# andimarafioti/faster-qwen3-tts

Measured on AMD Instinct MI355X. Metric: real-time factor (audio s / wall s), Qwen3-TTS-12Hz-0.6B voice-clone streaming chunk_size=8; p50 TTFA in ttfa_ms_p50, higher is better.
Workload: dtype bf16

## Files before the change

faster-qwen3-tts_amd/csrc/decode_kernels.cuh:

```cuda
#pragma once
#include "fq3_common.cuh"
#include <initializer_list>

namespace fq3 {

enum { PRO_PLAIN = 0, PRO_NORM = 1, PRO_COMBINE = 2 };
enum { EPI_STORE = 0, EPI_RESIDUAL = 1, EPI_SWIGLU = 2 };

constexpr int kHeadDim = 128;
constexpr int kKeysPerTile = 64;
constexpr int kMaxWorkers = 8;
constexpr int kPartStride = kHeadDim + 4;


struct GemvArgs {
    const void* W; int N; int K;
    const void* x;
    const void* norm_w; float eps;
    const void* bias;
    void* y;
    const void* res;
    void* xn_out;
    int up_off;
    const float* part; int n_part; int rep;
// ... 680 lines not shown
                       a.n_kv, a.rep, a.max_seq, a.pos_imm, attn_tail(a));
}

template <typename T>
__global__ __launch_bounds__(256) void rmsnorm_kernel(const T* x, const T* w, T* y, int K, float eps) {
    __shared__ float red[8];
    float ss = 0.f;
    for (int e = threadIdx.x; e < K; e += 256) { const float v = DT<T>::ld(x + e); ss = fmaf(v, v, ss); }
    ss = block_sum<4>(ss, red);
    const float rs = 1.0f / sqrtf(ss / (float)K + eps);
    for (int e = threadIdx.x; e < K; e += 256)
        DT<T>::st(y + e, DT<T>::ld(w + e) * DT<T>::rnd(DT<T>::ld(x + e) * rs));
}

template <typename T>
__global__ void copy_kernel(T* dst, const T* src, int n) {
    const int i = blockIdx.x * blockDim.x + threadIdx.x;
    if (i < n) dst[i] = src[i];
}

struct DecodeState {
    int token, frame, pos, gen_step, done;
    int text_open;
    int min_new, max_new, trailing_len, noise_frames, eos_id, max_seq, sup_lo, sup_hi;
    float t_temperature; int t_top_k; float t_top_p; int t_do_sample; float t_rep_penalty;
    float p_temperature; int p_top_k; float p_top_p; int p_do_sample;
    const void* trailing_text; const void* tts_pad; const void* talker_noise; const void* pred_noise;
    const void* past_hidden_init;
    int n_pad, rope_delta;
};

struct TeacherForcing { const int* forced; int* decisions; };

__device__ __forceinline__ int forced_or(const TeacherForcing* tf, int slot, int tok) {
    if (!tf) return tok;
    const int* forced = gptr(tf->forced); int* dec = gptr(tf->decisions);
    if (dec && threadIdx.x == 0) dec[slot] = tok;
    return forced ? forced[slot] : tok;
}

template <typename T>
__device__ __forceinline__ void frame_begin_body(DecodeState* st, const T* codec_emb, const T* past_hidden, T* ph_hold,
                                                 T* pred_in, int* codes, unsigned char* seen, int H, int G) {
    const int done = st->done;
    if (done == 1) return;
    const int tok = st->token;
    if (tok == st->eos_id || st->frame >= st->max_new) {
        __syncthreads();
        if (threadIdx.x == 0) st->done = 1;
        return;
    }
    if (st->text_open && st->gen_step >= st->trailing_len) {
        if (done == 0) {
            for (int e = threadIdx.x; e < H; e += 256) ph_hold[e] = past_hidden[e];
            __syncthreads();
            if (threadIdx.x == 0) st->done = 2;
        }
        return;
    }
    if (done == 2) {
        past_hidden = ph_hold;
        __syncthreads();
        if (threadIdx.x == 0) st->done = 0;
    }
    if (threadIdx.x == 0) { codes[(size_t)st->frame * G] = tok; seen[tok] = 1; }
    for (int e = threadIdx.x; e < H; e += 256) {
        pred_in[e] = past_hidden[e];
        pred_in[H + e] = codec_emb[(size_t)tok * H + e];
    }
}
// ... 72 lines not shown
```

faster-qwen3-tts_amd/csrc/fq3_api.hip:

```cpp
#define FQ3_SKINNY_EXTERN
#include "fq3_ctx.h"
#include "sampler.cuh"
#include "sampler_wave.cuh"
#include "skinny_gemm.cuh"
#include "state_kernels.cuh"

#include <cstdio>
#include <cstdlib>
#include <cstring>
#include <map>
#include <string>
#include <type_traits>
#include <vector>

using namespace fq3;

static thread_local std::string g_err;
static int fail(int code, const std::string& m) { g_err = m; return code; }
int fq3_fail_(int code, const std::string& m) { return fail(code, m); }
#define HIPCHK(x) do { hipError_t e_ = (x); if (e_ != hipSuccess) return fail(FQ3_EHIP, std::string(#x) + ": " + hipGetErrorString(e_)); } while (0)

extern "C" const char* fq3_last_error(void) { return g_err.c_str(); }
extern "C" void fq3_set_error_(const char* msg) { g_err = msg ? msg : ""; }
extern "C" int fq3_abi_version(void) { return FQ3_ABI_VERSION; }
// ... 190 lines not shown
    if ((r = dmalloc(c, &c->pred_x2, (size_t)p.hidden * c->esz))) return r;
    if ((r = dmalloc(c, &c->xin, (size_t)Hm * c->esz))) return r;
    if ((r = dmalloc(c, &c->tmp_hidden, (size_t)Hm * c->esz))) return r;
    if ((r = dmalloc(c, &c->qkv, (size_t)qkvm * c->esz))) return r;
    if ((r = dmalloc(c, &c->act, (size_t)Im * c->esz))) return r;
    if ((r = dmalloc(c, &c->logits, (size_t)Vm * c->esz))) return r;
    if ((r = dmalloc(c, &c->past_hidden, (size_t)t.hidden * c->esz))) return r;
    if ((r = dmalloc(c, &c->ph_hold, (size_t)t.hidden * c->esz))) return r;
    if ((r = dmalloc(c, &c->pred_in, (size_t)2 * t.hidden * c->esz))) return r;
    if ((r = dmalloc(c, &c->pred_next, (size_t)t.hidden * c->esz))) return r;
    if ((r = dmalloc(c, &c->pred_x, (size_t)p.hidden * c->esz))) return r;
    if ((r = dmalloc(c, &c->plogits, (size_t)(G - 1) * p.vocab * c->esz))) return r;
    const int maxkv = std::max(t.n_kv_heads, p.n_kv_heads);
    c->part_stride = (size_t)maxkv * kMaxWorkers * 4 * kPartStride;
    if ((r = dmalloc(c, (void**)&c->part, 2 * c->part_stride * sizeof(float)))) return r;
    if ((r = dmalloc(c, (void**)&c->rope_now, 2 * 64 * sizeof(float)))) return r;
    if ((r = dmalloc(c, (void**)&c->seen_api, kMaxVocab))) return r;
    if ((r = dmalloc(c, (void**)&c->st, sizeof(DecodeState)))) return r;
    if ((r = dmalloc(c, (void**)&c->seen, kMaxVocab))) return r;
    if ((r = dmalloc(c, (void**)&c->codes, (size_t)(frames + 1) * G * sizeof(int)))) return r;
    if ((r = dmalloc(c, (void**)&c->ids64, (size_t)64 * sizeof(int64_t)))) return r;
    if ((r = dmalloc(c, (void**)&c->d_pemb, (size_t)64 * sizeof(void*)))) return r;
    HIPCHK(hipStreamCreateWithFlags(&c->cap_stream, hipStreamNonBlocking));
    return FQ3_OK;
}

extern "C" int fq3_set_option(fq3_ctx* c, const char* key, int value) {
    if (!c || !key) return fail(FQ3_EINVAL, "null argument");
    const std::string k(key);
    if (k == "weight_nt") c->opt_nt = value;
    else if (k == "pred_m2") c->opt_m2 = value;
    else if (k == "pred_attn") c->opt_pred_attn = value;
    else if (k == "rows_per_wave_max") c->opt_rmax = value;
    else if (k == "prefill_mode") c->prefill_mode = value;
    else if (k == "flash_prefill") c->opt_flash_prefill = value;
    else if (k == "flash_small") c->opt_flash_small = value;
    else if (k == "cont_pack") c->opt_cont_pack = value;
    else if (k == "swiglu_tile") c->opt_swiglu_tile = value;
    else if (k == "packed_weights") c->opt_packed = value;
    else if (k == "skinny_gemm") c->opt_no_skinny = !value;
    else return fail(FQ3_EINVAL, "unknown option: " + k);
    fq3_graph_reset(c);
    return FQ3_OK;
}

extern "C" int fq3_graph_reset(fq3_ctx* c) {
    if (!c) return fail(FQ3_EINVAL, "null ctx");
    if (c->exec) { (void)hipGraphExecDestroy(c->exec); c->exec = nullptr; }
    if (c->graph) { (void)hipGraphDestroy(c->graph); c->graph = nullptr; }
    return FQ3_OK;
}

namespace {
struct PackedEntry { void* p; int refs; int N, K; };
std::mutex g_packed_mu;
std::map<std::pair<const void*, int>, PackedEntry> g_packed;
}
const void* fq3_packed_find_(const void* W, int kind) {
    std::lock_guard<std::mutex> lk(g_packed_mu);
    auto it = g_packed.find({W, kind});
    return it == g_packed.end() ? nullptr : it->second.p;
}
int fq3_packed_acquire_(const void* W, int N, int K, int kind) {
    if (!W || !skinny_pack_ok(N, K) || (kind == 1 && (N / 2) % 8) || (kind == 2 && N % 512)) return FQ3_EUNSUPPORTED;
    std::lock_guard<std::mutex> lk(g_packed_mu);
    auto it = g_packed.find({W, kind});
// ... 15 lines not shown
    if (it == g_packed.end()) return;
    if (--it->second.refs <= 0) { (void)hipFree(it->second.p); g_packed.erase(it); }
}
static void packed_release_all(fq3_ctx* c) {
    for (auto& r : c->packed_refs) fq3_packed_release_(r.first, r.second);
    c->packed_refs.clear();
}
static int packed_acquire_all(fq3_ctx* c) {
    if (c->cfg.dtype != FQ3_BF16) return FQ3_OK;
    auto take = [&](const void* W, int N, int K, int kind) -> int {
        const int r = fq3_packed_acquire_(W, N, K, kind);
        if (r == FQ3_OK) c->packed_refs.emplace_back(W, kind);
        return r == FQ3_EUNSUPPORTED ? FQ3_OK : r;
    };
    auto stack = [&](const std::vector<fq3_layer_weights>& L, const fq3_stack_dims& d) -> int {
        const int qd = d.n_heads * kHeadDim, kvd = d.n_kv_heads * kHeadDim;
        for (const fq3_layer_weights& l : L) {
            if (int r = take(l.qkv, qd + 2 * kvd, d.hidden, 0)) return r;
            if (int r = take(l.o, d.hidden, qd, 0)) return r;
            if (int r = take(l.gate_up, 2 * d.inter, d.hidden, 1)) return r;
            if (int r = take(l.gate_up, 2 * d.inter, d.hidden, 0)) return r;
            if (int r = take(l.down, d.hidden, d.inter, 0)) return r;
        }
        return FQ3_OK;
    };
    if (int r = stack(c->tl, c->cfg.talker)) return r;
    if (int r = stack(c->pl, c->cfg.predictor)) return r;
    for (const fq3_layer_weights& l : c->tl) if (int r = take(l.gate_up, 2 * c->cfg.talker.inter, c->cfg.talker.hidden, 2)) return r;
    if (int r = take(c->wt.codec_head, c->cfg.talker.vocab, c->cfg.talker.hidden, 0)) return r;
    for (const void* h : c->lmh) if (int r = take(h, c->cfg.predictor.vocab, c->cfg.predictor.hidden, 0)) return r;
    return FQ3_OK;
}

extern "C" int fq3_ctx_destroy(fq3_ctx* c) {
    if (!c) return FQ3_OK;
    (void)hipDeviceSynchronize();
    fq3_graph_reset(c);
    packed_release_all(c);
    if (c->cap_stream) (void)hipStreamDestroy(c->cap_stream);
    if (fq3_kv_pool* p = c->tk.pool) {
        (void)fq3_kv_release(c, 0);
        bool last;
        { std::lock_guard<std::mutex> lk(p->mu); last = --p->users == 0; }
        if (p->is_private && last) pool_free_(p);
    }
    for (void* p : c->allocs) (void)hipFree(p);
    delete c;
    return FQ3_OK;
}

extern "C" int fq3_bind_weights(fq3_ctx* c, const fq3_weight_table* w) {
    if (!c || !w) return fail(FQ3_EINVAL, "null argument");
    const int G = c->cfg.num_code_groups;
    if (!w->talker_layers || !w->predictor_layers || !w->codec_embedding || !w->codec_head || !w->talker_final_norm ||
        !w->predictor_final_norm || !w->predictor_embeddings || !w->lm_heads || !w->talker_cos || !w->talker_sin ||
        !w->pred_cos || !w->pred_sin)
        return fail(FQ3_EINVAL, "weight table has null entries");
    if (c->cfg.has_projection && !w->proj_w) return fail(FQ3_EINVAL, "has_projection set but proj_w is null");
    if (w->talker_rope_len < c->cfg.max_seq_len || w->pred_rope_len < G + 1)
        return fail(FQ3_EINVAL, "rope tables shorter than the caches");
    c->wt = *w;
    c->tl.assign(w->talker_layers, w->talker_layers + c->cfg.talker.n_layers);
    c->pl.assign(w->predictor_layers, w->predictor_layers + c->cfg.predictor.n_layers);
    c->pemb.assign(w->predictor_embeddings, w->predictor_embeddings + (G - 1));
    c->lmh.assign(w->lm_heads, w->lm_heads + (G - 1));
    for (auto& l : c->tl) if (!l.qkv || !l.o || !l.gate_up || !l.down || !l.input_norm || !l.post_norm || !l.q_norm || !l.k_norm)
        return fail(FQ3_EINVAL, "talker layer has null weights");
    for (auto& l : c->pl) if (!l.qkv || !l.o || !l.gate_up || !l.down || !l.input_norm || !l.post_norm || !l.q_norm || !l.k_norm)
        return fail(FQ3_EINVAL, "predictor layer has null weights");
    HIPCHK(hipMemcpy(c->d_pemb, c->pemb.data(), (G - 1) * sizeof(void*), hipMemcpyHostToDevice));
    (void)hipDeviceSynchronize();
    packed_release_all(c);
    if (int r = packed_acquire_all(c)) { packed_release_all(c); return r; }
    c->bound = true;
    fq3_graph_reset(c);
    return FQ3_OK;
}

template <typename T, int NCH, int PRO, int EPI, bool NT, int M = 1>
static void launch_gemv_n(const GemvArgs& a, int rmax, hipStream_t s) {
    const int R = gemv_rows_per_wave<NCH, EPI>(a.N, rmax);
    const int grid = gemv_grid(a.N, R);
    const size_t shm = gemv_lds_bytes<PRO, M>(a.K);
    if constexpr (MaxRows<NCH, EPI>::v >= 2) {
        if (R == 2) { gemv_launch<T, NCH, PRO, EPI, NT, M, 2>(a, grid, shm, s); return; }
    }
    gemv_launch<T, NCH, PRO, EPI, NT, M, 1>(a, grid, shm, s);
}
template <typename T, int PRO, int EPI>
static int launch_gemv2_t(const GemvArgs& a, int rmax, hipStream_t s) {
    constexpr int most = gemv_most_chunks(PRO, 2);
    const int n = gemv_chunks(a.K, most);
    if (!n) return fail(FQ3_EUNSUPPORTED, PRO == PRO_NORM ? "code predictor hidden size above 2048" : "code predictor GEMV inner dimension above 3072");
    with_value<1, 2, 4, 6>(n, [&](auto nch) {
        if constexpr (decltype(nch)::value <= most) launch_gemv_n<T, decltype(nch)::value, PRO, EPI, false, 2>(a, rmax, s);
    });
    return 0;
}
template <int PRO, int EPI>
static int launch_gemv2(const fq3_ctx* c, const GemvArgs& a, hipStream_t s) {
    return c->cfg.dtype == FQ3_BF16 ? launch_gemv2_t<bf16_t, PRO, EPI>(a, c->opt_rmax, s) : launch_gemv2_t<float, PRO, EPI>(a, c->opt_rmax, s);
}
template <typename T, int PRO, int EPI, bool NT>
static int launch_gemv_t(const GemvArgs& a, int rmax, hipStream_t s) {
    constexpr int most = gemv_most_chunks(PRO, 1);
    const int n = gemv_chunks(a.K, most);
    if (!n) return fail(FQ3_EUNSUPPORTED, PRO == PRO_NORM ? "hidden size above 2048" : "GEMV inner dimension above 6144");
    with_value<1, 2, 4, 6, 12>(n, [&](auto nch) {
        if constexpr (decltype(nch)::value <= most) launch_gemv_n<T, decltype(nch)::value, PRO, EPI, NT>(a, rmax, s);
    });
    return 0;
}
template <int PRO, int EPI>
static int launch_gemv(const fq3_ctx* c, const GemvArgs& a, bool nt, hipStream_t s) {
    const int rmax = c->opt_rmax;
    if (c->cfg.dtype == FQ3_BF16)
        return nt ? launch_gemv_t<bf16_t, PRO, EPI, true>(a, rmax, s) : launch_gemv_t<bf16_t, PRO, EPI, false>(a, rmax, s);
    return nt ? launch_gemv_t<float, PRO, EPI, true>(a, rmax, s) : launch_gemv_t<float, PRO, EPI, false>(a, rmax, s);
}

template <typename T, bool PAGED>
static void launch_attn_p(const AttnArgs& a, int rep, int workers, hipStream_t s) {
    with_value<1, 2, 4>(rep, [&](auto r) {
        attn_decode_launch<T, decltype(r)::value, PAGED>(a, workers, s);
    });
}
template <typename T>
static void launch_attn_t(const AttnArgs& a, int rep, int workers, hipStream_t s) {
    if (a.table) launch_attn_p<T, true>(a, rep, workers, s); else launch_attn_p<T, false>(a, rep, workers, s);
}

struct StepSrc { const void* x0; const int* pos_ptr; int pos_imm; bool kv_only_tail = false; };

static int run_stack(fq3_ctx* c, bool talker, const StepSrc& src, hipStream_t s) {
    const fq3_stack_dims& d = talker ? c->cfg.talker : c->cfg.predictor;
    const std::vector<fq3_layer_weights>& L = talker ? c->tl : c->pl;
    StackBufs& kv = talker ? c->tk : c->pk;
    const int rep = d.n_heads / d.n_kv_heads;
    const int q_dim = d.n_heads * kHeadDim, kv_dim = d.n_kv_heads * kHeadDim;
    const bool nt = c->opt_nt == 2 || (c->opt_nt == 1 && talker);
    const float *cos_row, *sin_row;
    if (src.pos_ptr) { cos_row = c->rope_now; sin_row = c->rope_now + 64; }
    else {
        const int rl = talker ? c->wt.talker_rope_len : c->wt.pred_rope_len;
        int rp = src.pos_imm + (talker ? c->rope_delta : 0);
        rp = rp < 0 ? 0 : (rp >= rl ? rl - 1 : rp);
        cos_row = (talker ? c->wt.talker_cos : c->wt.pred_cos) + (size_t)rp * 64;
        sin_row = (talker ? c->wt.talker_sin : c->wt.pred_sin) + (size_t)rp * 64;
    }
    for (int i = 0; i < d.n_layers; ++i) {
        const fq3_layer_weights& w = L[i];
        const void* xin = i == 0 ? src.x0 : c->h;
        GemvArgs g{};
        g.eps = d.rms_eps;
        g.W = w.qkv; g.N = q_dim + 2 * kv_dim; g.K = d.hidden; g.x = xin;
        g.norm_w = w.input_norm; g.y = c->qkv;
        if (int r = launch_gemv<PRO_NORM, EPI_STORE>(c, g, nt, s)) return r;
        const bool tail_skip = src.kv_only_tail && i == d.n_layers - 1;
        GemvArgs o{};
        o.W = w.o; o.N = d.hidden; o.K = q_dim; o.y = c->h; o.res = xin; o.rep = rep;
        AttnArgs a{};
        a.qkv = c->qkv; a.q_norm_w = w.q_norm; a.k_norm_w = w.k_norm; a.eps = d.rms_eps;
        a.cos_row = cos_row; a.sin_row = sin_row;
        a.kcache = kv.k[i]; a.vcache = kv.v[i]; a.max_seq = kv.max_seq;
        a.table = kv.d_table; a.blk_stride = kv.pool ? (int)kv.pool->blk_elems : 0;
        a.pos_ptr = src.pos_ptr; a.pos_imm = src.pos_imm;
        a.done_ptr = src.pos_ptr ? &c->st->done : nullptr;
        a.n_pad = talker ? c->n_pad : 0;
        a.n_kv = d.n_kv_heads; a.part = c->part;
        a.scale = 1.0f / sqrtf((float)kHeadDim);
        a.rep = rep; a.out = c->attn_out;
        const bool pred_attn = c->opt_pred_attn && !talker && !src.pos_ptr && src.pos_imm <= 16;
        if (pred_attn) {
            if (c->cfg.dtype == FQ3_BF16) attn_pred_launch<bf16_t>(a, d.n_heads, s);
            else attn_pred_launch<float>(a, d.n_heads, s);
            if (tail_skip) break;
            o.x = c->attn_out;
            if (int r = launch_gemv<PRO_PLAIN, EPI_RESIDUAL>(c, o, nt, s)) return r;
        } else {
            if (c->cfg.dtype == FQ3_BF16) launch_attn_t<bf16_t>(a, rep, kv.workers, s);
            else launch_attn_t<float>(a, rep, kv.workers, s);
            if (tail_skip) break;
            o.part = c->part; o.n_part = kv.workers;
            if (int r = launch_gemv<PRO_COMBINE, EPI_RESIDUAL>(c, o, nt, s)) return r;
        }
        GemvArgs m{};
        m.eps = d.rms_eps; m.W = w.gate_up; m.N = d.inter; m.K = d.hidden; m.x = c->h;
        m.norm_w = w.post_norm; m.y = c->act; m.up_off = d.inter;
        if (int r = launch_gemv<PRO_NORM, EPI_SWIGLU>(c, m, nt, s)) return r;
        GemvArgs dn{};
        dn.W = w.down; dn.N = d.hidden; dn.K = d.inter; dn.x = c->act; dn.y = c->h; dn.res = c->h;
        if (int r = launch_gemv<PRO_PLAIN, EPI_RESIDUAL>(c, dn, nt, s)) return r;
    }
    return 0;
}

static int run_predictor_pair(fq3_ctx* c, const void* x_a, const void* x_b, hipStream_t s) {
    const fq3_stack_dims& d = c->cfg.predictor;
    StackBufs& kv = c->pk;
    const int rep = d.n_heads / d.n_kv_heads;
    const int q_dim = d.n_heads * kHeadDim, kv_dim = d.n_kv_heads * kHeadDim;
    for (int i = 0; i < d.n_layers; ++i) {
        const fq3_layer_weights& w = c->pl[i];
        const void* xa = i == 0 ? x_a : c->h;
        const void* xb = i == 0 ? x_b : c->h2;
        GemvArgs g{};
        g.eps = d.rms_eps; g.W = w.qkv; g.N = q_dim + 2 * kv_dim; g.K = d.hidden; g.x = xa; g.x2 = xb;
        g.norm_w = w.input_norm; g.y = c->qkv; g.y2 = c->qkv2;
        if (int r = launch_gemv2<PRO_NORM, EPI_STORE>(c, g, s)) return r;
        for (int m = 0; m < 2; ++m) {
            AttnArgs a{};
            a.qkv = m == 0 ? c->qkv : c->qkv2; a.q_norm_w = w.q_norm; a.k_norm_w = w.k_norm; a.eps = d.rms_eps;
            a.cos_row = c->wt.pred_cos + (size_t)m * 64; a.sin_row = c->wt.pred_sin + (size_t)m * 64;
            a.kcache = kv.k[i]; a.vcache = kv.v[i]; a.max_seq = kv.max_seq;
            a.pos_ptr = nullptr; a.pos_imm = m; a.n_pad = 0; a.n_kv = d.n_kv_heads;
            a.part = c->part + (size_t)m * c->part_stride; a.scale = 1.0f / sqrtf((float)kHeadDim);
            a.rep = rep; a.out = m == 0 ? c->attn_out : c->attn_out2;
            if (c->opt_pred_attn) {
                if (c->cfg.dtype == FQ3_BF16) attn_pred_launch<bf16_t>(a, d.n_heads, s);
                else attn_pred_launch<float>(a, d.n_heads, s);
            } else if (c->cfg.dtype == FQ3_BF16) launch_attn_t<bf16_t>(a, rep, kv.workers, s);
            else launch_attn_t<float>(a, rep, kv.workers, s);
        }
        GemvArgs o{};
        o.W = w.o; o.N = d.hidden; o.K = q_dim; o.y = c->h; o.y2 = c->h2; o.res = xa; o.res2 = xb; o.rep = rep;
        if (c->opt_pred_attn) {
            o.x = c->attn_out; o.x2 = c->attn_out2;
// ... 327 lines not shown
                g_err = m;
                return r;
            }
    }
    if (walk) {
        for (int q = 0; q < n; ++q)
            if (int r = fq3_prefill_continue(ctxs[q], embeds[q], start[q], cnt[q], out_logits ? out_logits[q] : nullptr, out_hidden[q], stream)) return r;
        return FQ3_OK;
    }
    for (int q = 0; q < n; ++q)
        if (int r = fq3_set_generation_state(ctxs[q], 0, 0)) return r;
    if (int r = fq3_prefill_continue_batch_mfma_(ctxs, n, embeds, start, cnt, out_logits, out_hidden, s)) return r;
    LAUNCH_CHECK();
    return FQ3_OK;
}

int fq3_codec_head_launch_(fq3_ctx* c, const void* hidden, void* out_logits, hipStream_t s) {
    GemvArgs g{};
    g.W = c->wt.codec_head; g.N = c->cfg.talker.vocab; g.K = c->cfg.talker.hidden; g.x = hidden; g.y = out_logits;
    return launch_gemv<PRO_PLAIN, EPI_STORE>(c, g, true, s);
}

extern "C" int fq3_set_prefill_mode(fq3_ctx* c, int mode) { return fq3_set_option(c, "prefill_mode", mode); }

__global__ void build_seen_kernel(const int64_t* history, int n, unsigned char* seen, int V) {
    for (int i = threadIdx.x; i < V; i += blockDim.x) seen[i] = 0;
    __syncthreads();
    for (int i = threadIdx.x; i < n; i += blockDim.x) { const int id = (int)history[i]; if (id >= 0 && id < V) seen[id] = 1; }
}

template <typename T>
static void launch_sample_pred(const DecodeState* st, const T* lg, int V, int cb, const SampleCfg& cfg, const T* nz,
                               int* codes, int G, int64_t* out64, const T* next_emb, T* next_in, int H, bool wave,
                               const TeacherForcing* tf, hipStream_t s) {
    if (wave) dispatch_nc(V, [&](auto nc) {
        constexpr int NC = decltype(nc)::value;
        sample_pred_wave_launch<T, NC>(st, lg, V, cb, cfg, nz, codes, G, out64, next_emb, next_in, H, tf, s);
    });
    else hipLaunchKernelGGL((sample_pred_kernel<T>), dim3(1), dim3(256), 0, s, st, lg, V, cb, cfg, nz, codes, G, out64,
                            next_emb, next_in, H, tf);
}
template <typename T>
static void launch_sample_talker(DecodeState* st, const T* lg, int V, const unsigned char* seen, int G, bool wave,
                                 const TeacherForcing* tf, hipStream_t s) {
    if (wave) dispatch_nc(V, [&](auto nc) {
        constexpr int NC = decltype(nc)::value;
        sample_talker_wave_launch<T, NC>(st, lg, V, seen, G, tf, s);
    });
    else hipLaunchKernelGGL((sample_talker_kernel<T>), dim3(1), dim3(256), 0, s, st, lg, V, seen, G, tf);
}
template <typename T>
static void launch_sample_api(fq3_ctx* c, const T* lg, int V, const SampleCfg& cfg, const int64_t* history, int n_hist,
                              const T* noise, int64_t* out, hipStream_t s) {
    if (cfg.top_p >= 1.0f) {
        const unsigned char* seen = nullptr;
        if (n_hist > 0) {
            hipLaunchKernelGGL(build_seen_kernel, dim3(1), dim3(256), 0, s, history, n_hist, c->seen_api, V);
            seen = c->seen_api;
        }
        dispatch_nc(V, [&](auto nc) {
            constexpr int NC = decltype(nc)::value;
            hipLaunchKernelGGL((sample_api_wave_kernel<T, NC>), dim3(1), dim3(256), 0, s, lg, V, cfg, seen, noise, out);
        });
    } else {
        hipLaunchKernelGGL((sample_api_kernel<T>), dim3(1), dim3(256), 0, s, lg, V, cfg, history, n_hist, noise, out);
    }
}

static SampleCfg to_cfg(const fq3_sampling& s) {
    SampleCfg c{};
// ... 26 lines not shown
    for (int i = threadIdx.x; i < V; i += 256) {
        if (!seen[i]) continue;
        const float v = DT<T>::ld(logits + i);
        DT<T>::st(logits + i, v > 0.f ? v / penalty : v * penalty);
    }
}
extern "C" int fq3_apply_repetition_penalty(fq3_ctx* c, void* logits, int V, const int64_t* history, int n_hist,
                                            float penalty, void* stream) {
    if (!c || !logits) return fail(FQ3_EINVAL, "null argument");
    if (V <= 0 || V > kMaxVocab) return fail(FQ3_EUNSUPPORTED, "vocab must be at most 4096");
    if (penalty == 1.0f || n_hist <= 0 || !history) return FQ3_OK;
    hipStream_t s = (hipStream_t)stream;
    hipLaunchKernelGGL(build_seen_kernel, dim3(1), dim3(256), 0, s, history, n_hist, c->seen_api, V);
    if (c->cfg.dtype == FQ3_BF16) hipLaunchKernelGGL((rep_penalty_kernel<bf16_t>), dim3(1), dim3(256), 0, s, (bf16_t*)logits, V, c->seen_api, penalty);
    else hipLaunchKernelGGL((rep_penalty_kernel<float>), dim3(1), dim3(256), 0, s, (float*)logits, V, c->seen_api, penalty);
    LAUNCH_CHECK();
    return FQ3_OK;
}

extern "C" int fq3_set_predictor_sampling(fq3_ctx* c, const fq3_sampling* s) {
    if (!c || !s) return fail(FQ3_EINVAL, "null argument");
    if (s->do_sample && !(s->temperature > 0.f)) return fail(FQ3_EINVAL, "temperature must be > 0");
    if ((s->top_p >= 1.0f) != (c->pred_sampling.top_p >= 1.0f)) fq3_graph_reset(c);
    c->pred_sampling = *s;
    return FQ3_OK;
}

template <typename T>
static int predictor_passes_t(fq3_ctx* c, const DecodeState* st_dev, const void* pred_input, const void* noise_imm,
                              int64_t* out64, void* out_logits, hipStream_t s) {
    const fq3_stack_dims &p = c->cfg.predictor, &t = c->cfg.talker;
    const int G = c->cfg.num_code_groups, Vp = p.vocab, Ht = t.hidden;
    SampleCfg scfg = to_cfg(c->pred_sampling);
    for (int pass = 0; pass < G; ++pass) {
        const void* hsrc = c->h;
        if (pass == 0 && c->opt_m2) {
            const T* xa = (const T*)pred_input;
            const T* xb = (const T*)pred_input + Ht;
            if (c->cfg.has_projection) {
                GemvArgs g{};
                g.W = c->wt.proj_w; g.bias = c->wt.proj_b; g.N = p.hidden; g.K = Ht; g.x = xa; g.x2 = xb; g.y = c->pred_x; g.y2 = c->pred_x2;
                if (int r = launch_gemv2<PRO_PLAIN, EPI_STORE>(c, g, s)) return r;
                xa = (const T*)c->pred_x; xb = (const T*)c->pred_x2;
            }
            if (int r = run_predictor_pair(c, xa, xb, s)) return r;
            pass = 1;
            hsrc = c->h2;
        } else {
        const T* x_talker = pass < 2 ? (const T*)pred_input + (size_t)pass * Ht : (const T*)c->pred_next;
        const void* x0 = x_talker;
        if (c->cfg.has_projection) {
            GemvArgs g{};
            g.W = c->wt.proj_w; g.bias = c->wt.proj_b; g.N = p.hidden; g.K = Ht; g.x = x_talker; g.y = c->pred_x;
            if (int r = launch_gemv<PRO_PLAIN, EPI_STORE>(c, g, false, s)) return r;
            x0 = c->pred_x;
        }
        StepSrc src{x0, nullptr, pass};
        src.kv_only_tail = pass == 0;
        if (int r = run_stack(c, false, src, s)) return r;
        }
        if (pass == 0) continue;
        const int cb = pass - 1;
        T* lg = out_logits ? (T*)out_logits + (size_t)cb * Vp : (T*)c->plogits + (size_t)cb * Vp;
        GemvArgs hgm{};
        hgm.eps = p.rms_eps; hgm.W = c->lmh[cb]; hgm.N = Vp; hgm.K = p.hidden; hgm.x = hsrc;
        hgm.norm_w = c->wt.predictor_final_norm; hgm.y = lg;
        if (int r = launch_gemv<PRO_NORM, EPI_STORE>(c, hgm, false, s)) return r;
        const T* nz = noise_imm ? (const T*)noise_imm + (size_t)cb * Vp : nullptr;
        const T* next_emb = cb + 1 < G - 1 ? (const T*)c->pemb[cb] : nullptr;
        launch_sample_pred<T>(st_dev, (const T*)lg, Vp, cb, scfg, nz, st_dev ? c->codes : nullptr, G, out64, next_emb,
                              (T*)c->pred_next, Ht, c->pred_sampling.top_p >= 1.0f, st_dev ? c->tf : nullptr, s);
    }
    return 0;
}

extern "C" int fq3_predictor_loop(fq3_ctx* c, const void* pred_input, const void* noise, int64_t* out_ids,
                                  void* out_logits, void* stream) {
    NEED_BOUND(c);
    if (!pred_input || !out_ids) return fail(FQ3_EINVAL, "null argument");
    if (c->pred_sampling.do_sample && !noise) return fail(FQ3_EINVAL, "predictor sampling enabled but no noise given");
    hipStream_t s = (hipStream_t)stream;
    int r = c->cfg.dtype == FQ3_BF16 ? predictor_passes_t<bf16_t>(c, nullptr, pred_input, noise, out_ids, out_logits, s)
                                     : predictor_passes_t<float>(c, nullptr, pred_input, noise, out_ids, out_logits, s);
    if (r) return r;
    LAUNCH_CHECK();
    return FQ3_OK;
}

extern "C" int fq3_decode_begin(fq3_ctx* c, const fq3_decode_params* p, void* stream) {
    NEED_BOUND(c);
    if (!p || !p->past_hidden || !p->tts_pad_embed) return fail(FQ3_EINVAL, "null argument");
    if (p->trailing_len > 0 && !p->trailing_text) return fail(FQ3_EINVAL, "trailing_text");
    if (p->talker.do_sample && (!p->talker_noise || p->noise_frames <= 0)) return fail(FQ3_EINVAL, "talker sampling needs a noise ring");
    if (c->pred_sampling.do_sample && (!p->pred_noise || p->noise_frames <= 0)) return fail(FQ3_EINVAL, "predictor sampling needs a noise ring");
    if (p->talker.do_sample && !(p->talker.temperature > 0.f)) return fail(FQ3_EINVAL, "temperature must be > 0");
    if (p->max_new_tokens > c->cfg.max_frames) return fail(FQ3_EINVAL, "max_new_tokens exceeds the context's max_frames");
    if (p->prefill_len <= 0 || p->prefill_len > c->cfg.max_seq_len) return fail(FQ3_EINVAL, "prefill_len");
    if (p->first_token < 0 || p->first_token >= c->cfg.talker.vocab) return fail(FQ3_EINVAL, "first_token outside the codec vocabulary");
    if (p->gen_step < 0 || p->min_new_tokens < 0 || p->max_new_tokens < 0) return fail(FQ3_EINVAL, "negative counters");
    const bool wave = p->talker.top_p >= 1.0f;
    if (wave != c->talker_wave) { fq3_graph_reset(c); c->talker_wave = wave; }
    hipStream_t s = (hipStream_t)stream;
    if (int r = fq3_kv_ensure_(c, p->prefill_len + p->max_new_tokens + 1, s)) return r;
    DecodeState h{};
// ... 114 lines not shown
```

faster-qwen3-tts_amd/csrc/fq3_ctx.h:

```cpp
#pragma once
#include "../../include/fq3hip.h"
#include "decode_kernels.cuh"
#include <hip/hip_runtime.h>
#include <mutex>
#include <string>
#include <utility>
#include <vector>

struct fq3_kv_pool {
    int dtype = 0, esz = 2, n_layers = 0, n_kv = 0, n_blocks = 0;
    size_t blk_elems = 0;
    std::vector<void*> k, v;
    std::vector<int> free_list;
    std::mutex mu;
    int in_use_high = 0;
    int users = 0;
    bool is_private = false;
};

struct StackBufs {
    std::vector<void*> k, v;
    int max_seq = 0, workers = 1;
    fq3_kv_pool* pool = nullptr;
    int* d_table = nullptr;
    std::vector<int> blocks;
    int max_blocks = 0;
};

struct fq3_ctx {
    fq3_config cfg{};
    int esz = 2;
    std::vector<fq3_layer_weights> tl, pl;
    fq3_weight_table wt{};
    std::vector<const void*> pemb, lmh;
    const void** d_pemb = nullptr;
    bool bound = false;
    StackBufs tk, pk;
    void *h = nullptr, *xin = nullptr, *qkv = nullptr, *act = nullptr, *logits = nullptr, *past_hidden = nullptr;
    void *pred_in = nullptr, *pred_x = nullptr, *pred_next = nullptr, *plogits = nullptr, *tmp_hidden = nullptr;
    void *attn_out = nullptr, *attn_out2 = nullptr;
    void *h2 = nullptr, *qkv2 = nullptr, *act2 = nullptr, *pred_x2 = nullptr;
    size_t part_stride = 0;
    float* part = nullptr;
    float* rope_now = nullptr;
    unsigned char* seen_api = nullptr;
    fq3::DecodeState* st = nullptr;
    fq3::TeacherForcing* tf = nullptr;
    unsigned char* seen = nullptr;
    int* codes = nullptr;
    int64_t* ids64 = nullptr;
    int n_pad = 0, rope_delta = 0;
    int opt_nt = 1;
    int opt_m2 = 1;
    int opt_pred_attn = 1;
    int opt_rmax = 2;
    int opt_flash_prefill = 1;
    int opt_flash_small = 1;
    int opt_cont_pack = 1;
    int opt_swiglu_tile = 1;
    int opt_packed = 1;
    std::vector<std::pair<const void*, int>> packed_refs;
    int opt_no_skinny = 0;
    int prefill_mode = 0;
    bool talker_wave = true;
    fq3_sampling pred_sampling{0.9f, 50, 1.0f, 1, 1.0f};
    hipGraph_t graph = nullptr;
    hipGraphExec_t exec = nullptr;
    hipStream_t cap_stream = nullptr;
    std::vector<void*> allocs;
    fq3_prompt_weights pw{};
    bool pw_bound = false;
    void *pw_x = nullptr, *pw_h = nullptr;
    int pw_cap = 0;
    void* ph_hold = nullptr;
    void *tt_tab = nullptr, *tt_x = nullptr, *tt_h = nullptr;
    int tt_alloc = 0;
    int tt_cap = 0, tt_rows = 0;
    bool tt_open = false, tt_session = false;
    bool armed = false;
    const void* begin_trailing = nullptr; int begin_trailing_len = 0;
    void *pf_x = nullptr, *pf_xn = nullptr, *pf_qkv = nullptr, *pf_att = nullptr, *pf_gu = nullptr, *pf_act = nullptr, *pf_ws = nullptr;
};


const void* fq3_packed_find_(const void* W, int kind);
int fq3_packed_acquire_(const void* W, int N, int K, int kind);
void fq3_packed_release_(const void* W, int kind);

// ... 13 lines not shown
```

faster-qwen3-tts_amd/csrc/sampler_wave.cuh:

```cuda
#pragma once
#include "sampler.cuh"
#include <type_traits>

namespace fq3 {

__device__ __forceinline__ ArgMax wave_argmax(ArgMax a) {
    ArgMax r;
    r.v = wave_max(a.v);
    r.i = wave_min_i32(a.v == r.v ? a.i : 0x7fffffff);
    return r;
}

struct BlkSmem { int cnt[2][4]; float f[4]; float av[4]; int ai[4]; };

__device__ __forceinline__ float blk_max4(float v, BlkSmem& sm) {
    v = wave_max(v);
    __syncthreads();
    if ((threadIdx.x & 63) == 0) sm.f[threadIdx.x >> 6] = v;
    __syncthreads();
    return fmaxf(fmaxf(sm.f[0], sm.f[1]), fmaxf(sm.f[2], sm.f[3]));
}
__device__ __forceinline__ float blk_sum4(float v, BlkSmem& sm) {
    v = wave_sum(v);
    __syncthreads();
// ... 125 lines not shown
        if (off < V) ldraw<false>(xraw[j], logits + off); else zero(xraw[j]);
    }
}

template <typename T, int NC>
__global__ __launch_bounds__(256) void sample_api_wave_kernel(const T* logits, int V, SampleCfg c, const unsigned char* seen,
                                                             const T* noise, int64_t* out) {
    __shared__ BlkSmem sm;
    Raw8<T> xraw[NC];
    issue_logits<T, NC>(xraw, logits, V);
    const int tok = sample_wave_core<T, NC>(xraw, V, c, seen, noise, sm);
    if (threadIdx.x == 0) out[0] = tok;
}

template <typename T, int NC>
__device__ __forceinline__ int sample_nucleus_from_regs(Raw8<T> (&xraw)[NC], int V, const SampleCfg& c, const unsigned char* seen,
                                                        const T* noise, SampleSmem& big) {
#pragma unroll
    for (int j = 0; j < NC; ++j) {
        float f[8];
        unpack(xraw[j], f);
#pragma unroll
        for (int i = 0; i < 8; ++i) {
            const int id = j * 2048 + threadIdx.x * 8 + i;
            if (id < V) big.vals[id] = f[i];
        }
    }
    __syncthreads();
    const int tok = sample_core<T>(big, V, c, seen, noise);
    __syncthreads();
    return tok;
}

template <typename T, int NC, bool NUCLEUS = false>
__device__ __forceinline__ void sample_pred_wave_body(const DecodeState* st, const T* logits, int V, int cb,
                                                      const SampleCfg& c_imm, const T* noise_imm, int* codes, int G,
                                                      int64_t* out64, const T* next_emb, T* next_in, int H, const TeacherForcing* tf = nullptr) {
    __shared__ BlkSmem sm;
    Raw8<T> xraw[NC];
    issue_logits<T, NC>(xraw, logits, V);
    SampleCfg c = c_imm;
    const T* noise = noise_imm;
    int frame = 0;
    if (st) {
        if (st->done) return;
        c.temperature = st->p_temperature; c.top_k = st->p_top_k; c.top_p = st->p_top_p; c.do_sample = st->p_do_sample;
        frame = st->frame;
        if (st->pred_noise)
            noise = gptr(reinterpret_cast<const T*>(st->pred_noise)) + ((size_t)(frame % st->noise_frames) * (G - 1) + cb) * V;
    }
    int tok;
    if constexpr (NUCLEUS) {
        __shared__ SampleSmem big;
        if (c.do_sample && c.top_p < 1.0f) tok = sample_nucleus_from_regs<T, NC>(xraw, V, c, nullptr, noise, big);
        else tok = sample_wave_core<T, NC>(xraw, V, c, nullptr, noise, sm);
    } else {
        tok = sample_wave_core<T, NC>(xraw, V, c, nullptr, noise, sm);
    }
    if (st) tok = forced_or(tf, frame * G + 1 + cb, tok);
    if (threadIdx.x == 0) {
        if (codes) codes[(size_t)frame * G + 1 + cb] = tok;
        if (out64) out64[cb] = tok;
    }
    if (next_emb) {
        const T* src = next_emb + (size_t)tok * H;
        for (int e = threadIdx.x * 8; e < H; e += 256 * 8) {
            Raw8<T> r; ldraw<false>(r, src + e);
            if (sizeof(T) == 2) *reinterpret_cast<u32x4*>(reinterpret_cast<char*>(next_in) + (size_t)e * 2) = *reinterpret_cast<u32x4*>(&r);
            else { float f[8]; unpack(r, f);
#pragma unroll
                   for (int i = 0; i < 8; ++i) DT<T>::st(next_in + e + i, f[i]); }
        }
    }
}

constexpr int kSamplePredLeadDwords = 14;
template <typename T, int NC>
__global__ __launch_bounds__(256) void sample_pred_wave_kernel(const DecodeState* st, const T* logits, const T* noise_imm, int* codes,
                                                              int64_t* out64, const T* next_emb, int V, int cb, int G, int H,
                                                              T* next_in, const TeacherForcing* tf, SampleCfg c_imm) {
    sample_pred_wave_body<T, NC>(st, logits, V, cb, c_imm, noise_imm, codes, G, out64, next_emb, next_in, H, tf);
}
template <typename T, int NC>
inline void sample_pred_wave_launch(const DecodeState* st, const T* logits, int V, int cb, const SampleCfg& c_imm, const T* noise_imm,
                                    int* codes, int G, int64_t* out64, const T* next_emb, T* next_in, int H, const TeacherForcing* tf,
                                    hipStream_t s) {
    hipLaunchKernelGGL((sample_pred_wave_kernel<T, NC>), dim3(1), dim3(256), 0, s, st, logits, noise_imm, codes, out64, next_emb, V, cb, G, H,
                       next_in, tf, c_imm);
}

template <typename T, int NC, bool NUCLEUS = false>
__device__ __forceinline__ void sample_talker_wave_body(DecodeState* st, const T* logits, int V, const unsigned char* seen, int G,
                                                        const TeacherForcing* tf = nullptr) {
    __shared__ BlkSmem sm;
    Raw8<T> xraw[NC];
    issue_logits<T, NC>(xraw, logits, V);
    if (st->done) return;
    SampleCfg c;
    c.temperature = st->t_temperature; c.top_k = st->t_top_k; c.top_p = st->t_top_p; c.do_sample = st->t_do_sample;
    c.rep_penalty = st->t_rep_penalty;
    c.sup_lo = st->sup_lo; c.sup_hi = st->sup_hi; c.keep_id = st->eos_id;
    const int frame = st->frame;
    c.sup_extra = (frame + 1 < st->min_new) ? st->eos_id : -1;
    const T* noise = st->talker_noise
        ? gptr(reinterpret_cast<const T*>(st->talker_noise)) + (size_t)(frame % st->noise_frames) * V : nullptr;
    int tok;
    if constexpr (NUCLEUS) {
        __shared__ SampleSmem big;
        if (c.do_sample && c.top_p < 1.0f) tok = sample_nucleus_from_regs<T, NC>(xraw, V, c, seen, noise, big);
        else tok = sample_wave_core<T, NC>(xraw, V, c, seen, noise, sm);
    } else {
        tok = sample_wave_core<T, NC>(xraw, V, c, seen, noise, sm);
    }
    tok = forced_or(tf, (frame + 1) * G, tok);
    if (threadIdx.x == 0) { st->token = tok; st->frame = frame + 1; st->pos += 1; st->gen_step += 1; }
}
constexpr int kSampleTalkerLeadDwords = 10;
template <typename T, int NC>
__global__ __launch_bounds__(256) void sample_talker_wave_kernel(DecodeState* st, const T* logits, const unsigned char* seen,
                                                                const TeacherForcing* tf, int V, int G) {
    sample_talker_wave_body<T, NC>(st, logits, V, seen, G, tf);
// ... 9 lines not shown
```

Baseline: 39.13.

## Precompute predictor layer-0 QKV table per codebook token and fuse sampling with entry attention

Builds a shared per-weight table holding the projected input and the layer-0 normed QKV output for every codebook token id. At predictor passes ≥2 the sampler gathers the sampled token's row directly, so the projection GEMV and the layer-0 QKV GEMV are skipped. Optionally, a fused kernel runs sampling in every head block and then layer-0 attention on the gathered row, removing a launch. This costs a large device table (groups × vocab × qkv width) and a build step at weight binding, and it duplicates sampling work across blocks.

```diff
diff --git a/faster-qwen3-tts_amd/csrc/decode_kernels.cuh b/faster-qwen3-tts_amd/csrc/decode_kernels.cuh
--- a/faster-qwen3-tts_amd/csrc/decode_kernels.cuh
+++ b/faster-qwen3-tts_amd/csrc/decode_kernels.cuh
@@ -736,10 +736,10 @@
 
 struct TeacherForcing { const int* forced; int* decisions; };
 
-__device__ __forceinline__ int forced_or(const TeacherForcing* tf, int slot, int tok) {
+__device__ __forceinline__ int forced_or(const TeacherForcing* tf, int slot, int tok, bool record = true) {
     if (!tf) return tok;
     const int* forced = gptr(tf->forced); int* dec = gptr(tf->decisions);
-    if (dec && threadIdx.x == 0) dec[slot] = tok;
+    if (dec && record && threadIdx.x == 0) dec[slot] = tok;
     return forced ? forced[slot] : tok;
 }
 
diff --git a/faster-qwen3-tts_amd/csrc/fq3_api.hip b/faster-qwen3-tts_amd/csrc/fq3_api.hip
--- a/faster-qwen3-tts_amd/csrc/fq3_api.hip
+++ b/faster-qwen3-tts_amd/csrc/fq3_api.hip
@@ -246,6 +246,8 @@
     else if (k == "pred_m2") c->opt_m2 = value;
     else if (k == "pred_attn") c->opt_pred_attn = value;
     else if (k == "rows_per_wave_max") c->opt_rmax = value;
+    else if (k == "pred_table") c->opt_pred_table = value;
+    else if (k == "pred_entry_attn") c->opt_pred_entry_attn = value;
     else if (k == "prefill_mode") c->prefill_mode = value;
     else if (k == "flash_prefill") c->opt_flash_prefill = value;
     else if (k == "flash_small") c->opt_flash_small = value;
@@ -327,11 +329,15 @@
     return FQ3_OK;
 }
 
+static void pred_table_acquire(fq3_ctx* c);
+static void pred_table_release(fq3_ctx* c);
+
 extern "C" int fq3_ctx_destroy(fq3_ctx* c) {
     if (!c) return FQ3_OK;
     (void)hipDeviceSynchronize();
     fq3_graph_reset(c);
     packed_release_all(c);
+    pred_table_release(c);
     if (c->cap_stream) (void)hipStreamDestroy(c->cap_stream);
     if (fq3_kv_pool* p = c->tk.pool) {
         (void)fq3_kv_release(c, 0);
@@ -366,7 +372,9 @@
     HIPCHK(hipMemcpy(c->d_pemb, c->pemb.data(), (G - 1) * sizeof(void*), hipMemcpyHostToDevice));
     (void)hipDeviceSynchronize();
     packed_release_all(c);
+    pred_table_release(c);
     if (int r = packed_acquire_all(c)) { packed_release_all(c); return r; }
+    pred_table_acquire(c);
     c->bound = true;
     fq3_graph_reset(c);
     return FQ3_OK;
@@ -425,7 +433,83 @@
     if (a.table) launch_attn_p<T, true>(a, rep, workers, s); else launch_attn_p<T, false>(a, rep, workers, s);
 }
 
-struct StepSrc { const void* x0; const int* pos_ptr; int pos_imm; bool kv_only_tail = false; };
+struct StepSrc { const void* x0; const int* pos_ptr; int pos_imm; bool kv_only_tail = false; bool qkv0_ready = false; bool attn0_ready = false; };
+
+namespace {
+struct PredTabEntry { void* qkv; void* res; int refs; };
+std::mutex g_ptab_mu;
+std::map<std::vector<uint64_t>, PredTabEntry> g_ptab;
+}
+static bool pred_table_build(fq3_ctx* c, PredTabEntry& e) {
+    const fq3_stack_dims &p = c->cfg.predictor, &t = c->cfg.talker;
+    const int n_tab = c->cfg.num_code_groups - 2, Vp = p.vocab, Ht = t.hidden, Hp = p.hidden;
+    const int N = (p.n_heads + 2 * p.n_kv_heads) * kHeadDim;
+    const bool proj = c->cfg.has_projection != 0;
+    e = PredTabEntry{nullptr, nullptr, 0};
+    if (n_tab < 1 || (!proj && Ht != Hp)) return false;
+    const size_t rows = (size_t)n_tab * Vp;
+    hipStream_t s = nullptr;
+    bool ok = hipMalloc(&e.qkv, rows * N * c->esz) == hipSuccess && (!proj || hipMalloc(&e.res, rows * Hp * c->esz) == hipSuccess) &&
+              hipStreamCreateWithFlags(&s, hipStreamNonBlocking) == hipSuccess;
+    for (int cb = 0; ok && cb < n_tab; ++cb)
+        for (int id = 0; ok && id < Vp; ++id) {
+            const size_t row = (size_t)cb * Vp + id;
+            const void* x = (const char*)c->pemb[cb] + (size_t)id * Ht * c->esz;
+            if (proj) {
+                GemvArgs g{};
+                g.W = c->wt.proj_w; g.bias = c->wt.proj_b; g.N = Hp; g.K = Ht; g.x = x; g.y = (char*)e.res + row * Hp * c->esz;
+                ok = launch_gemv<PRO_PLAIN, EPI_STORE>(c, g, false, s) == 0;
+                x = g.y;
+            }
+            GemvArgs g{};
+            g.eps = p.rms_eps; g.W = c->pl[0].qkv; g.N = N; g.K = Hp; g.x = x; g.norm_w = c->pl[0].input_norm;
+            g.y = (char*)e.qkv + row * N * c->esz;
+            ok = ok && launch_gemv<PRO_NORM, EPI_STORE>(c, g, false, s) == 0;
+        }
+    if (s) { ok = hipStreamSynchronize(s) == hipSuccess && ok; (void)hipStreamDestroy(s); }
+    if (!ok) {
+        (void)hipGetLastError();
+        if (e.qkv) (void)hipFree(e.qkv);
+        if (e.res) (void)hipFree(e.res);
+        e = PredTabEntry{nullptr, nullptr, 0};
+    }
+    return ok;
+}
+static void pred_table_release(fq3_ctx* c) {
+    c->ptab_qkv = c->ptab_res = nullptr;
+    if (c->ptab_key.empty()) return;
+    std::lock_guard<std::mutex> lk(g_ptab_mu);
+    auto it = g_ptab.find(c->ptab_key);
+    if (it != g_ptab.end() && --it->second.refs <= 0) {
+        (void)hipFree(it->second.qkv);
+        if (it->second.res) (void)hipFree(it->second.res);
+        g_ptab.erase(it);
+    }
+    c->ptab_key.clear();
+}
+static void pred_table_acquire(fq3_ctx* c) {
+    const fq3_stack_dims &p = c->cfg.predictor, &t = c->cfg.talker;
+    const int n_tab = c->cfg.num_code_groups - 2;
+    int dev = 0;
+    (void)hipGetDevice(&dev);
+    uint32_t eps_bits;
+    memcpy(&eps_bits, &p.rms_eps, sizeof eps_bits);
+    std::vector<uint64_t> key{(uint64_t)(uintptr_t)c->pl[0].qkv, (uint64_t)(uintptr_t)c->pl[0].input_norm, (uint64_t)(uintptr_t)c->wt.proj_w,
+                              (uint64_t)(uintptr_t)c->wt.proj_b, (uint64_t)c->cfg.dtype, (uint64_t)c->cfg.has_projection, (uint64_t)p.vocab,
+                              (uint64_t)t.hidden, (uint64_t)p.hidden, (uint64_t)p.n_heads, (uint64_t)p.n_kv_heads, (uint64_t)n_tab,
+                              (uint64_t)eps_bits, (uint64_t)dev};
+    for (int cb = 0; cb < n_tab; ++cb) key.push_back((uint64_t)(uintptr_t)c->pemb[cb]);
+    std::lock_guard<std::mutex> lk(g_ptab_mu);
+    auto it = g_ptab.find(key);
+    if (it == g_ptab.end()) {
+        PredTabEntry e;
+        if (!pred_table_build(c, e)) return;
+        it = g_ptab.emplace(key, e).first;
+    }
+    ++it->second.refs;
+    c->ptab_key = std::move(key);
+    c->ptab_qkv = it->second.qkv; c->ptab_res = it->second.res;
+}
 
 static int run_stack(fq3_ctx* c, bool talker, const StepSrc& src, hipStream_t s) {
     const fq3_stack_dims& d = talker ? c->cfg.talker : c->cfg.predictor;
@@ -450,7 +534,8 @@
         g.eps = d.rms_eps;
         g.W = w.qkv; g.N = q_dim + 2 * kv_dim; g.K = d.hidden; g.x = xin;
         g.norm_w = w.input_norm; g.y = c->qkv;
-        if (int r = launch_gemv<PRO_NORM, EPI_STORE>(c, g, nt, s)) return r;
+        if (!(i == 0 && src.qkv0_ready))
+            if (int r = launch_gemv<PRO_NORM, EPI_STORE>(c, g, nt, s)) return r;
         const bool tail_skip = src.kv_only_tail && i == d.n_layers - 1;
         GemvArgs o{};
         o.W = w.o; o.N = d.hidden; o.K = q_dim; o.y = c->h; o.res = xin; o.rep = rep;
@@ -467,7 +552,8 @@
         a.rep = rep; a.out = c->attn_out;
         const bool pred_attn = c->opt_pred_attn && !talker && !src.pos_ptr && src.pos_imm <= 16;
         if (pred_attn) {
-            if (c->cfg.dtype == FQ3_BF16) attn_pred_launch<bf16_t>(a, d.n_heads, s);
+            if (i == 0 && src.attn0_ready) {}
+            else if (c->cfg.dtype == FQ3_BF16) attn_pred_launch<bf16_t>(a, d.n_heads, s);
             else attn_pred_launch<float>(a, d.n_heads, s);
             if (tail_skip) break;
             o.x = c->attn_out;
@@ -488,6 +574,20 @@
         if (int r = launch_gemv<PRO_PLAIN, EPI_RESIDUAL>(c, dn, nt, s)) return r;
     }
     return 0;
+}
+
+static AttnArgs pred_layer0_attn_args(fq3_ctx* c, int pos) {
+    const fq3_stack_dims& d = c->cfg.predictor;
+    const fq3_layer_weights& w = c->pl[0];
+    const int rp = pos < 0 ? 0 : (pos >= c->wt.pred_rope_len ? c->wt.pred_rope_len - 1 : pos);
+    AttnArgs a{};
+    a.qkv = c->qkv; a.q_norm_w = w.q_norm; a.k_norm_w = w.k_norm; a.eps = d.rms_eps;
+    a.cos_row = c->wt.pred_cos + (size_t)rp * 64; a.sin_row = c->wt.pred_sin + (size_t)rp * 64;
+    a.kcache = c->pk.k[0]; a.vcache = c->pk.v[0]; a.max_seq = c->pk.max_seq;
+    a.pos_imm = pos; a.n_kv = d.n_kv_heads; a.part = c->part;
+    a.scale = 1.0f / sqrtf((float)kHeadDim);
+    a.rep = d.n_heads / d.n_kv_heads; a.out = c->attn_out;
+    return a;
 }
 
 static int run_predictor_pair(fq3_ctx* c, const void* x_a, const void* x_b, hipStream_t s) {
@@ -881,10 +981,10 @@
 template <typename T>
 static void launch_sample_pred(const DecodeState* st, const T* lg, int V, int cb, const SampleCfg& cfg, const T* nz,
                                int* codes, int G, int64_t* out64, const T* next_emb, T* next_in, int H, bool wave,
-                               const TeacherForcing* tf, hipStream_t s) {
+                               const TeacherForcing* tf, hipStream_t s, const T* qkv_tab = nullptr, T* qkv_out = nullptr, int qkv_n = 0) {
     if (wave) dispatch_nc(V, [&](auto nc) {
         constexpr int NC = decltype(nc)::value;
-        sample_pred_wave_launch<T, NC>(st, lg, V, cb, cfg, nz, codes, G, out64, next_emb, next_in, H, tf, s);
+        sample_pred_wave_launch<T, NC>(st, lg, V, cb, cfg, nz, codes, G, out64, next_emb, next_in, H, tf, s, qkv_tab, qkv_out, qkv_n);
     });
     else hipLaunchKernelGGL((sample_pred_kernel<T>), dim3(1), dim3(256), 0, s, st, lg, V, cb, cfg, nz, codes, G, out64,
                             next_emb, next_in, H, tf);
@@ -977,6 +1077,10 @@
     const fq3_stack_dims &p = c->cfg.predictor, &t = c->cfg.talker;
     const int G = c->cfg.num_code_groups, Vp = p.vocab, Ht = t.hidden;
     SampleCfg scfg = to_cfg(c->pred_sampling);
+    const bool wave = c->pred_sampling.top_p >= 1.0f;
+    const bool tab = c->opt_pred_table && c->ptab_qkv && wave;
+    const bool entry = tab && c->opt_pred_entry_attn && c->opt_pred_attn && G - 1 <= 16;
+    const int Hp = p.hidden, qkv_n = (p.n_heads + 2 * p.n_kv_heads) * kHeadDim;
     for (int pass = 0; pass < G; ++pass) {
         const void* hsrc = c->h;
         if (pass == 0 && c->opt_m2) {
@@ -994,14 +1098,18 @@
         } else {
         const T* x_talker = pass < 2 ? (const T*)pred_input + (size_t)pass * Ht : (const T*)c->pred_next;
         const void* x0 = x_talker;
+        const bool from_tab = tab && pass >= 2;
         if (c->cfg.has_projection) {
             GemvArgs g{};
             g.W = c->wt.proj_w; g.bias = c->wt.proj_b; g.N = p.hidden; g.K = Ht; g.x = x_talker; g.y = c->pred_x;
-            if (int r = launch_gemv<PRO_PLAIN, EPI_STORE>(c, g, false, s)) return r;
+            if (!from_tab)
+                if (int r = launch_gemv<PRO_PLAIN, EPI_STORE>(c, g, false, s)) return r;
             x0 = c->pred_x;
         }
         StepSrc src{x0, nullptr, pass};
         src.kv_only_tail = pass == 0;
+        src.qkv0_ready = from_tab;
+        src.attn0_ready = from_tab && entry;
         if (int r = run_stack(c, false, src, s)) return r;
         }
         if (pass == 0) continue;
@@ -1013,8 +1121,24 @@
         if (int r = launch_gemv<PRO_NORM, EPI_STORE>(c, hgm, false, s)) return r;
         const T* nz = noise_imm ? (const T*)noise_imm + (size_t)cb * Vp : nullptr;
         const T* next_emb = cb + 1 < G - 1 ? (const T*)c->pemb[cb] : nullptr;
+        T* next_in = (T*)c->pred_next;
+        int next_h = Ht;
+        const T* qkv_tab = nullptr;
+        if (tab && next_emb) {
+            const size_t row0 = (size_t)cb * Vp;
+            qkv_tab = (const T*)c->ptab_qkv + row0 * qkv_n;
+            if (c->cfg.has_projection) { next_emb = (const T*)c->ptab_res + row0 * Hp; next_in = (T*)c->pred_x; next_h = Hp; }
+        }
+        if (entry && qkv_tab) {
+            const AttnArgs a0 = pred_layer0_attn_args(c, pass + 1);
+            dispatch_nc(Vp, [&](auto nc) {
+                sample_pred_entry_launch<T, decltype(nc)::value>(st_dev, (const T*)lg, Vp, cb, scfg, nz, st_dev ? c->codes : nullptr, G, out64, next_emb,
+                                                                 next_in, next_h, st_dev ? c->tf : nullptr, qkv_tab, qkv_n, a0, p.n_heads, s);
+            });
+            continue;
+        }
         launch_sample_pred<T>(st_dev, (const T*)lg, Vp, cb, scfg, nz, st_dev ? c->codes : nullptr, G, out64, next_emb,
-                              (T*)c->pred_next, Ht, c->pred_sampling.top_p >= 1.0f, st_dev ? c->tf : nullptr, s);
+                              next_in, next_h, wave, st_dev ? c->tf : nullptr, s, qkv_tab, (T*)c->qkv, qkv_n);
     }
     return 0;
 }
diff --git a/faster-qwen3-tts_amd/csrc/fq3_ctx.h b/faster-qwen3-tts_amd/csrc/fq3_ctx.h
--- a/faster-qwen3-tts_amd/csrc/fq3_ctx.h
+++ b/faster-qwen3-tts_amd/csrc/fq3_ctx.h
@@ -54,6 +54,10 @@
     int opt_m2 = 1;
     int opt_pred_attn = 1;
     int opt_rmax = 2;
+    int opt_pred_table = 1;
+    int opt_pred_entry_attn = 1;
+    std::vector<uint64_t> ptab_key;
+    const void *ptab_qkv = nullptr, *ptab_res = nullptr;
     int opt_flash_prefill = 1;
     int opt_flash_small = 1;
     int opt_cont_pack = 1;
diff --git a/faster-qwen3-tts_amd/csrc/sampler_wave.cuh b/faster-qwen3-tts_amd/csrc/sampler_wave.cuh
--- a/faster-qwen3-tts_amd/csrc/sampler_wave.cuh
+++ b/faster-qwen3-tts_amd/csrc/sampler_wave.cuh
@@ -181,10 +181,22 @@
     return tok;
 }
 
+template <typename T>
+__device__ __forceinline__ void gather_row(const T* src, T* dst, int n) {
+    for (int e = threadIdx.x * 8; e < n; e += 256 * 8) {
+        Raw8<T> r; ldraw<false>(r, src + e);
+        if (sizeof(T) == 2) *reinterpret_cast<u32x4*>(reinterpret_cast<char*>(dst) + (size_t)e * 2) = *reinterpret_cast<u32x4*>(&r);
+        else { float f[8]; unpack(r, f);
+#pragma unroll
+               for (int i = 0; i < 8; ++i) DT<T>::st(dst + e + i, f[i]); }
+    }
+}
+
 template <typename T, int NC, bool NUCLEUS = false>
 __device__ __forceinline__ void sample_pred_wave_body(const DecodeState* st, const T* logits, int V, int cb,
                                                       const SampleCfg& c_imm, const T* noise_imm, int* codes, int G,
-                                                      int64_t* out64, const T* next_emb, T* next_in, int H, const TeacherForcing* tf = nullptr) {
+                                                      int64_t* out64, const T* next_emb, T* next_in, int H, const TeacherForcing* tf = nullptr,
+                                                      const T* qkv_tab = nullptr, T* qkv_out = nullptr, int qkv_n = 0) {
     __shared__ BlkSmem sm;
     Raw8<T> xraw[NC];
     issue_logits<T, NC>(xraw, logits, V);
@@ -211,31 +223,70 @@
         if (codes) codes[(size_t)frame * G + 1 + cb] = tok;
         if (out64) out64[cb] = tok;
     }
-    if (next_emb) {
-        const T* src = next_emb + (size_t)tok * H;
-        for (int e = threadIdx.x * 8; e < H; e += 256 * 8) {
-            Raw8<T> r; ldraw<false>(r, src + e);
-            if (sizeof(T) == 2) *reinterpret_cast<u32x4*>(reinterpret_cast<char*>(next_in) + (size_t)e * 2) = *reinterpret_cast<u32x4*>(&r);
-            else { float f[8]; unpack(r, f);
-#pragma unroll
-                   for (int i = 0; i < 8; ++i) DT<T>::st(next_in + e + i, f[i]); }
-        }
-    }
+    if (next_emb) gather_row<T>(next_emb + (size_t)tok * H, next_in, H);
+    if (qkv_tab) gather_row<T>(qkv_tab + (size_t)tok * qkv_n, qkv_out, qkv_n);
 }
 
 constexpr int kSamplePredLeadDwords = 14;
 template <typename T, int NC>
 __global__ __launch_bounds__(256) void sample_pred_wave_kernel(const DecodeState* st, const T* logits, const T* noise_imm, int* codes,
                                                               int64_t* out64, const T* next_emb, int V, int cb, int G, int H,
-                                                              T* next_in, const TeacherForcing* tf, SampleCfg c_imm) {
-    sample_pred_wave_body<T, NC>(st, logits, V, cb, c_imm, noise_imm, codes, G, out64, next_emb, next_in, H, tf);
+                                                              T* next_in, const TeacherForcing* tf, SampleCfg c_imm, const T* qkv_tab,
+                                                              T* qkv_out, int qkv_n) {
+    sample_pred_wave_body<T, NC>(st, logits, V, cb, c_imm, noise_imm, codes, G, out64, next_emb, next_in, H, tf, qkv_tab, qkv_out, qkv_n);
 }
 template <typename T, int NC>
 inline void sample_pred_wave_launch(const DecodeState* st, const T* logits, int V, int cb, const SampleCfg& c_imm, const T* noise_imm,
                                     int* codes, int G, int64_t* out64, const T* next_emb, T* next_in, int H, const TeacherForcing* tf,
-                                    hipStream_t s) {
+                                    hipStream_t s, const T* qkv_tab = nullptr, T* qkv_out = nullptr, int qkv_n = 0) {
     hipLaunchKernelGGL((sample_pred_wave_kernel<T, NC>), dim3(1), dim3(256), 0, s, st, logits, noise_imm, codes, out64, next_emb, V, cb, G, H,
-                       next_in, tf, c_imm);
+                       next_in, tf, c_imm, qkv_tab, qkv_out, qkv_n);
+}
+
+struct PredEntryTail {
+    SampleCfg c_imm; int G, H; void* next_in; const TeacherForcing* tf; const void* qkv_tab; int qkv_n;
+    void* kcache; void* vcache; int n_kv, max_seq, pos_imm;
+    AttnTail at;
+};
+constexpr int kSamplePredEntryLeadDwords = 14;
+template <typename T, int NC>
+__global__ __launch_bounds__(256) void sample_pred_entry_kernel(const DecodeState* st, const T* logits, const T* noise_imm, int* codes,
+                                                               int64_t* out64, const T* next_emb, int V, int cb, PredEntryTail t) {
+    __shared__ BlkSmem sm;
+    Raw8<T> xraw[NC];
+    issue_logits<T, NC>(xraw, logits, V);
+    SampleCfg c = t.c_imm;
+    const T* noise = noise_imm;
+    const bool writer = blockIdx.x == 0;
+    int frame = 0;
+    if (st) {
+        if (st->done) return;
+        c.temperature = st->p_temperature; c.top_k = st->p_top_k; c.top_p = st->p_top_p; c.do_sample = st->p_do_sample;
+        frame = st->frame;
+        if (st->pred_noise)
+            noise = gptr(reinterpret_cast<const T*>(st->pred_noise)) + ((size_t)(frame % st->noise_frames) * (t.G - 1) + cb) * V;
+    }
+    int tok = sample_wave_core<T, NC>(xraw, V, c, nullptr, noise, sm);
+    if (st) tok = forced_or(t.tf, frame * t.G + 1 + cb, tok, writer);
+    if (writer) {
+        if (threadIdx.x == 0) {
+            if (codes) codes[(size_t)frame * t.G + 1 + cb] = tok;
+            if (out64) out64[cb] = tok;
+        }
+        if (next_emb) gather_row<T>(next_emb + (size_t)tok * t.H, reinterpret_cast<T*>(t.next_in), t.H);
+    }
+    if (threadIdx.x >= 64) return;
+    AttnArgs a = attn_args_of(t.at);
+    a.qkv = reinterpret_cast<const T*>(t.qkv_tab) + (size_t)tok * t.qkv_n;
+    a.kcache = t.kcache; a.vcache = t.vcache; a.n_kv = t.n_kv; a.max_seq = t.max_seq; a.pos_imm = t.pos_imm;
+    attn_pred_body<T>(a, (int)blockIdx.x);
+}
+template <typename T, int NC>
+inline void sample_pred_entry_launch(const DecodeState* st, const T* logits, int V, int cb, const SampleCfg& c_imm, const T* noise_imm,
+                                     int* codes, int G, int64_t* out64, const T* next_emb, T* next_in, int H, const TeacherForcing* tf,
+                                     const T* qkv_tab, int qkv_n, const AttnArgs& a, int heads, hipStream_t s) {
+    const PredEntryTail t{c_imm, G, H, next_in, tf, qkv_tab, qkv_n, a.kcache, a.vcache, a.n_kv, a.max_seq, a.pos_imm, attn_tail(a)};
+    hipLaunchKernelGGL((sample_pred_entry_kernel<T, NC>), dim3(heads), dim3(256), 0, s, st, logits, noise_imm, codes, out64, next_emb, V, cb, t);
 }
 
 template <typename T, int NC, bool NUCLEUS = false>
```

After: 40.00 (median of 6 runs). 1.02x the previous value.
